# IIT-PAVIS/DiffAssemble

Hardware: AMD Instinct MI355X
Metric: denoising steps/sec (900-piece dense graph, T=100) (higher is better)
Workload: dtype bf16

## Files before the change

diffassemble_amd/_lib.py:

```python
import ctypes as C
import os

import torch

LIB_PATH = os.environ.get("DA_LIB_PATH") or os.path.join(os.path.dirname(os.path.abspath(__file__)), "lib", "libdiffassemble_hip.so")
DA_MAX_LAYERS = 8
ABI_VERSION = 19
PREC_F32, PREC_BF16 = 0, 1
VARIANT_2D, VARIANT_3D, VARIANT_DISCRETE = 0, 1, 2
ARCH_TRANSFORMER, ARCH_EXOPHORMER, ARCH_GCN = 0, 1, 2
MEAN_EPSILON, MEAN_START_X = 0, 1
ACT_NONE, ACT_GELU, ACT_LEAKY02 = 0, 1, 2
CONV_Q_PRESCALED, CONV_FOLDED_V32 = 1, 2
TRAIN_MMA_FP32, TRAIN_MMA_BF16 = 0, 1
TRAIN_BWD_ALL, TRAIN_BWD_EARLY, TRAIN_BWD_LATE = 0, 1, 2
D3PM_DRAW_SAMPLING, D3PM_DRAW_TRAINING = 0, 1
D3PM_LOSS = {"vb": 0, "cross_entropy": 1, "hybrid": 2}
DBG_COUNTERS = ("opt_gen_workgroups", "dense_fast_exits", "dual_gen_slabs", "opt_masked_gen_workgroups")
DBG_LAUNCH_COUNTERS = {"resident_launches": 4, "virtual_rows_in_launch": 5}
PROF_CLASSES = ("embed", "linear_mlp", "linear_qkvs", "attn_hidden", "attn_last", "head", "update", "conv_fused")

_fp = C.c_void_p
_FPL = _fp * DA_MAX_LAYERS


class DaWeights(C.Structure):
    _fields_ = [
        ("variant", C.c_int32), ("arch", C.c_int32), ("steps", C.c_int32), ("c_in", C.c_int32),
        ("c_out", C.c_int32), ("feat_dim", C.c_int32), ("hidden", C.c_int32), ("heads", C.c_int32),
        ("n_layers", C.c_int32), ("virt_nodes", C.c_int32),
        ("time_emb", _fp),
        ("pos_w0", _fp), ("pos_b0", _fp), ("pos_w1", _fp), ("pos_b1", _fp),
        ("mlp_w0", _fp), ("mlp_b0", _fp), ("mlp_w1", _fp), ("mlp_b1", _fp),
        ("conv_wq", _FPL), ("conv_bq", _FPL), ("conv_wk", _FPL), ("conv_bk", _FPL),
# ... 285 lines not shown
```

diffassemble_amd/csrc/da_api.hip:

```cpp
#include <stdarg.h>
#include <stdlib.h>
#include <string.h>

#include <utility>
#include <vector>

#include "da_common.h"
#include "da_internal.h"
#include "da_config.h"

namespace da {

static thread_local char g_err[1024] = "";

void set_error(const char *fmt, ...) {
    va_list ap;
    va_start(ap, fmt);
    vsnprintf(g_err, sizeof(g_err), fmt, ap);
    va_end(ap);
}

struct ConvW {
    void *w = nullptr;
    float *b = nullptr;
// ... 55 lines not shown
    float *mlp_b0 = nullptr, *mlp_b1 = nullptr;
    ConvW conv[DA_MAX_LAYERS];
    void *virt_emb = nullptr;
    void *head_w0 = nullptr;
    float *head_b0 = nullptr;
    float *head_w1 = nullptr, *head_b1 = nullptr, *head_r_w1 = nullptr, *head_r_b1 = nullptr;
    bool fused_mlp2 = false;
    void *conv0c_w = nullptr;
    float *conv0c_b = nullptr;
    void *headc_w = nullptr;
    float *headc_b = nullptr;
    void *virt_qkvs = nullptr;
    void *conv0c_wd = nullptr, *virt_qkvs_d = nullptr;
    void *conv0c_wdp = nullptr, *convLf_wp = nullptr;
    void *conv0c_wqs = nullptr;
    float *conv0c_bd = nullptr;
    bool q_prescaled = false;
    bool lastfold = false;
    bool dense_only = false;
    void *convLf_w = nullptr;
    float *convLf_b = nullptr;
    void *skipc_w = nullptr;
    float *skipc_b = nullptr;
    std::vector<void *> owned;
    bool prof_on = false;
    std::vector<hipEvent_t> prof_ev;
    std::vector<int> prof_cls;
    size_t prof_used = 0;
    struct LoopEntry { LoopKey a, b; hipGraphExec_t exec, exec_b; };
    std::vector<LoopEntry> loops;
// ... 332 lines not shown
                        DA_CHECK_HIP(hipStreamWaitEvent(st, d->ev_join, 0));
                        side_guard.armed = false;
                        xin = dst; ldx = c.hc;
                        continue;
                    }
                    rc = timed(d, last ? DA_PROF_ATTN_LAST : DA_PROF_ATTN_HIDDEN, st, [&] {
                        int r2 = launch_attn_dense(prec, L, d->heads, c.C, g->n_graphs, g->max_graph_nodes, g->graph_ptr,
                                                   g->pad_ptr, 0, resid, act, dst, st, &mk);
                        if (r2) return r2;
                        return launch_attn_csr_cont(prec, n, nr, g->agg_row_ptr ? g->agg_row_ptr : g->irr_row_ptr, g->agg_row_ptr ? g->agg_col_src : g->irr_col_src,
                                                    g->row_map, d->heads, c.C, g->n_pad, L, resid, act, dst, st, g->agg_row_ptr ? g->agg_mult : nullptr); });
                    if (rc) return rc < 0 ? 1 : rc;
                    xin = dst; ldx = c.hc;
                    continue;
                }
                rc = timed(d, last ? DA_PROF_ATTN_LAST : DA_PROF_ATTN_HIDDEN, st, [&] {
                    return launch_attn_dense(prec, L, d->heads, c.C, g->n_graphs, g->max_graph_nodes, g->graph_ptr,
                                             g->pad_ptr, g->dense == 2, resid, act, dst, st); });
                if (rc > 0) return rc;
                if (rc == 0) { xin = dst; ldx = c.hc; continue; }
            }
        }
        if ((rc = timed(d, DA_PROF_LINEAR_QKVS, st, [&] {
                 return linear(prec, nproj, c.din, 4 * c.hc, xin, ldx, c.w, c.b, DA_ACT_NONE, nullptr, w.qkvs, 4 * c.hc, st); }))) return rc;
        if (virt0 && (rc = launch_scatter_virtual(prec, n - nr, d->V, d->heads, c.C, d->virt_qkvs, nr, nullptr, 0, nullptr, nullptr,
                                                  nullptr, nullptr, w.qkvs, st))) return rc;
        DA_REQUIRE(g->row_ptr && (g->col_src || g->n_edges == 0), "da_graph: this call walks the edge list (alpha requested or no "
                   "MFMA attention for this layer) but the CSR arrays are missing");
        int tiny = -1;
        if (!al && g->dense && n == nr && g->graph_ptr && !dense_disabled()) {
            if ((rc = timed(d, last ? DA_PROF_ATTN_LAST : DA_PROF_ATTN_HIDDEN, st, [&] {
// ... 163 lines not shown
        void *p = nullptr;
        if (hipMalloc(&p, bytes < 256 ? 256 : bytes) != hipSuccess) { set_error("hipMalloc(%zu) failed", bytes); return nullptr; }
        d->owned.push_back(p);
        return p;
    };
    auto copy_f32 = [&](const float *src, size_t n) -> float * {
        float *p = (float *)alloc(n * 4);
        if (!p || hipMemcpyAsync(p, src, n * 4, hipMemcpyDeviceToDevice, st) != hipSuccess) { rc = 2; return nullptr; }
        return p;
    };
    auto pack = [&](const float *src, size_t n) -> void * {
        void *p = alloc(n * s + 4096);
        if (!p || launch_convert(precision, n, src, p, st)) { rc = 2; return nullptr; }
        return p;
    };
    auto pack_qs = [&](const void *wsrc, int K, int hc, int C) -> void * {
#ifndef DA_EXPERIMENTS
        return nullptr;
#endif
        if (precision != DA_PREC_BF16 || C != 32 || H != 8 || (K != 128 && K != 256) || !wsrc || mfma_disabled()) return nullptr;
        void *p = alloc(w_qs_bytes(H, K));
        if (!p || pack_w_qs(H, K, hc, wsrc, p, st)) { rc = 2; return nullptr; }
        return p;
    };
    auto pack_panel = [&](const void *wsrc, int K, int Nout) -> void * {
        const size_t nb = xpanel_in_model() ? da_linear_packed_bytes(precision, K, Nout) : 0;
        if (!nb || !wsrc) return nullptr;
        void *p = alloc(nb);
        if (!p || pack_w_xpanel(K, Nout, wsrc, K, p, st)) { rc = 2; return nullptr; }
        return p;
    };
    d->time_emb = copy_f32(w->time_emb, (size_t)w->steps * 32);
    if (discrete) {
        d->pos_w1 = copy_f32(w->pos_w1, (size_t)w->c_out * 32);
// ... 549 lines not shown
int da_conv_dense_ex(int prec, const da_graph *g, int heads, int C, int Din, const void *x, const void *w, const float *b,
                     const void *residual, int act, void *out, void *scratch, int flags, void *stream) {
    DA_REQUIRE(g && x && w && out && scratch, "da_conv_dense_ex: null argument");
    DA_REQUIRE(dense_ok(g, heads, C), "da_conv_dense_ex: graph is not dense or head width %d unsupported", C);
    const bool folded = (flags & DA_CONV_FOLDED_V32) != 0;
    DA_REQUIRE(!folded || (C == 144 && !residual && act == DA_ACT_NONE), "da_conv_dense_ex: folded value heads need C = 144, no residual, no activation");
    hipStream_t st = (hipStream_t)stream;
    const size_t s = esize(prec), hc = (size_t)heads * C;
    const size_t hb = align_up(((size_t)g->n_pad + 64) * hc * s, 256);
    char *base = (char *)scratch;
    QkvScatter qs;
    qs.HC = (int)hc; qs.C = C; qs.n_pad = g->n_pad; qs.row_map = g->row_map;
    qs.Q = base; qs.K = base + hb; qs.Vt = base + 2 * hb; qs.S = folded ? nullptr : base + 3 * hb;
    qs.Cv = folded ? 32 : 0;
    const int nout = folded ? 2 * (int)hc + heads * 32 : 4 * (int)hc;
    const bool qsf = !folded && !residual && !g->hybrid && g->n_nodes == g->n_real && b && w_qs_bytes(heads, Din) <= hb &&
                     attn_qsf_applicable(prec, heads, C, Din, g->n_graphs, g->max_graph_nodes, g->n_pad, (flags & DA_CONV_Q_PRESCALED) ? 1 : 0);
    void *wq_img = base + hb;
    int rc = 0;
    if (qsf) {
        if ((rc = pack_w_qs(heads, Din, (int)hc, w, wq_img, st))) return rc;
    } else
    rc = launch_gemm_mfma(prec, g->n_nodes, Din, nout, x, Din, w, b, DA_ACT_NONE, nullptr, nullptr, 0, &qs, st);
    DA_REQUIRE(rc == 0, "da_conv_dense_ex: projection shape (Din=%d, Nout=%d) not supported by the MFMA kernels", Din, nout);
    DenseLayout L;
    L.Q = qs.Q; L.K = qs.K; L.Vt = qs.Vt; L.S = qs.S; L.n_pad = g->n_pad; L.q_prescaled = (flags & DA_CONV_Q_PRESCALED) ? 1 : 0;
    if (qsf) { L.x = x; L.ldx = Din; L.kin = Din; L.wqs = wq_img; L.bias = b; }
    DenseFold fo;
    fo.cv = 32; fo.out = out; fo.n_rows = g->n_real;
    const DenseMask mk = dense_mask_of(g);
    rc = launch_attn_dense(prec, L, heads, C, g->n_graphs, g->max_graph_nodes, g->graph_ptr, g->pad_ptr, g->dense == 2, residual, act,
// ... 4 lines not shown

int da_debug_counters(int64_t *out, int n, int reset) {
    DA_REQUIRE(out && n >= DA_DBG_NCOUNTERS, "da_debug_counters: need room for %d counters", DA_DBG_NCOUNTERS);
    unsigned long long a[4] = {0, 0, 0, 0}, b2[2] = {0, 0};
    int rc;
    if ((rc = da::attn_dense_counters(a, reset))) return rc;
#ifdef DA_EXPERIMENTS
    if ((rc = da::attn_dual_counters(b2, reset))) return rc;
#endif
    for (int k = 0; k < n; ++k) out[k] = 0;
    out[DA_DBG_OPT_GEN_WORKGROUPS] = (int64_t)a[0];
    out[DA_DBG_DENSE_FAST_EXITS] = (int64_t)a[1];
    out[DA_DBG_DUAL_GEN_SLABS] = (int64_t)b2[0];
    out[DA_DBG_OPT_MASKED_GEN_WORKGROUPS] = (int64_t)a[2];
    out[DA_DBG_RES_LAUNCHES] = (int64_t)da::attn_res_launches(reset);
    out[DA_DBG_VIRT_IN_LAUNCH] = (int64_t)da::attn_virt_launches(reset);
    return 0;
}

int da_profile_enable(da_denoiser *d, int on) {
    DA_REQUIRE(d, "da_profile_enable: null denoiser");
    d->prof_on = on != 0;
    d->prof_used = 0;
    d->prof_cls.clear();
    return 0;
}

int da_profile_read(da_denoiser *d, float *ms, int32_t *counts) {
    DA_REQUIRE(d && ms && counts, "da_profile_read: null argument");
    for (int k = 0; k < DA_PROF_NCLASS; ++k) { ms[k] = 0.f; counts[k] = 0; }
// ... 54 lines not shown
```

diffassemble_amd/csrc/da_attn_dense.hip:

```cpp
#include <stdlib.h>

#include "da_attn_common.h"

namespace da {

#ifdef DA_ATTN_PROBE
#define DA_ATTN_DBG(...) __VA_ARGS__
#define DA_TICK(var) const unsigned long long var = __builtin_readcyclecounter()
#else
#define DA_ATTN_DBG(...)
#define DA_TICK(var)
#endif

__device__ unsigned long long g_attn_fallbacks[4];

template <typename T, int C, bool MASKED, int CV, int NST, int NW>
__global__ __launch_bounds__(64 * NW, (sizeof(T) == 4 && C == 144 && CV == 144) ? 1 : 2) void k_attn_dense(AttnDenseParams p) {
    using CF = Cfg<T, C, CV>;
    constexpr int QT = 32 * NW, NT = 64 * NW, MAXI = (CF::NI + NW - 1) / NW;
    extern __shared__ __attribute__((aligned(16))) unsigned char smem[];

    float *mlut = (float *)(smem + NST * CF::STAGE);
    if (MASKED && threadIdx.x < 64) {
        const int e = threadIdx.x >> 2, b = threadIdx.x & 3;
// ... 743 lines not shown
#ifdef DA_EXPERIMENTS
    if (prec == DA_PREC_BF16 && C == 32 && !p.mask && attn2_env() DA_ATTN_DBG(&& !p.debug && !p.prof))
        return launch_attn_dense2(p, heads, n_graphs, max_graph_nodes, st);
#endif
    if (prec == DA_PREC_BF16) return C == 32 ? launch_tc<bf16_t, 32>(p, st) : launch_tc<bf16_t, 144>(p, st);
    return C == 32 ? launch_tc<float, 32>(p, st) : launch_tc<float, 144>(p, st);
}

bool attn_res_qsf_shape_ok(int max_nodes, int n_pad, int n_graphs, int kin);
bool attn_qsf_applicable(int prec, int heads, int C, int kin, int n_graphs, int max_graph_nodes, int n_pad, int q_prescaled) {
    if (prec != DA_PREC_BF16 || heads != 8 || C != 32 || !q_prescaled || !attn_opt_env()) return false;
    if (DA_XENV("DA_ATTN_NO_FAST", 0) DA_ATTN_DBG(|| DA_XENV_LIVE("DA_ATTN_DEBUG") || DA_XENV_LIVE("DA_ATTN_PROF_PTR"))) return false;
    if ((size_t)C * (size_t)n_pad * 2 >= ((size_t)1 << 31)) return false;
    return attn_res_qsf_shape_ok(max_graph_nodes, n_pad, n_graphs, kin);
}

int attn_dense_counters(unsigned long long *out4, int reset) {
    DA_CHECK_HIP(hipMemcpyFromSymbol(out4, HIP_SYMBOL(g_attn_fallbacks), 4 * sizeof(unsigned long long)));
    if (reset) { const unsigned long long z[4] = {0, 0, 0, 0}; DA_CHECK_HIP(hipMemcpyToSymbol(HIP_SYMBOL(g_attn_fallbacks), z, sizeof(z))); }
    unsigned long long o2[2] = {0, 0};
    const int rc = attn_opt_counters(o2, reset);
    if (rc) return rc;
    out4[0] = o2[0];
    out4[2] = o2[1];
    return 0;
}

}
```

diffassemble_amd/csrc/da_attn_opt.hip:

```cpp
#include <stdlib.h>

#include <type_traits>

#include "da_attn_common.h"
#include "da_attn_res_asm.inc"

namespace da {

#ifdef DA_OPT_PROBE
#define DA_OPB(...) __VA_ARGS__
#else
#define DA_OPB(...)
#endif

__device__ unsigned long long g_opt_fallbacks[2];

__device__ __forceinline__ void virt_rows_block(const AttnDenseParams &p, int vb, unsigned char *smem) {
    constexpr int EPL = 4, U = 4, C = 32;
    const int row = vb / p.v_split, part = vb - row * p.v_split;
    const int i = p.v_n_real + row;
    const int beg = p.v_row_ptr[i], end = p.v_row_ptr[i + 1];
    const int lane = threadIdx.x & 63, wv = threadIdx.x >> 6;
    const int head = lane >> 3, sub = (lane & 7) * EPL;
    const size_t hb = (size_t)head * (size_t)p.n_pad;
// ... 722 lines not shown
    int grid = p.nqt * p.H * p.n_graphs;
    t_virt_taken = false;
    if constexpr (C == 32 && !FOLD && MASKED && NWV == 4) {
        if (p.v_rows > 0) {
            p.v_split = p.v_n_real >= 8192 ? DA_VIRT_SPLIT_MAX : 4;
            grid += (p.v_rows * p.v_split + 7) & ~7;
            t_virt_taken = true;
            __atomic_fetch_add(&g_virt_launches, 1ll, __ATOMIC_RELAXED);
        }
    } else {
        p.v_rows = 0;
    }
    k_attn_optt<C, FOLD, MASKED, NST, MINB, BK, VAR, NWV><<<grid, 64 * NWV, lds, st>>>(p);
    DA_LAUNCH_CHECK();
    return 0;
}

template <int NWV, bool QUEUE, bool KPF, int XV = 0>
__global__ __launch_bounds__(64 * NWV, NWV >= 16 ? 1 : ((NWV > 5 || (XV & 8)) ? 4 : 5)) void k_attn_res(AttnDenseParams p) {
    constexpr bool O2 = (XV & 1) != 0, PROG = (XV & 16) != 0, MSK = (XV & 32) != 0, QSF = (XV & 64) != 0, PIPE2 = (XV & 256) != 0;
    static_assert(!PIPE2 || (NWV == 16 && KPF && !PROG && !MSK && !O2), "pipelined key loop: the sixteen-wave instances on complete graphs");
    static_assert(!QSF || (NWV == 16 && KPF && QUEUE && !PROG && !MSK && !O2), "projection in the prologue: the sixteen-wave default instance");
    static_assert(!MSK || (NWV == 16 && KPF && !PROG && !O2), "masked resident instance: sixteen waves, K fragments one block ahead");
    static_assert(!PROG || (NWV == 16 && KPF), "progressive landing: the sixteen-wave instance (two waves per piece index), K fragments one block ahead");
    using T = bf16_t;
    constexpr int C = 32, CV = 32;
    using CF = Cfg<T, C, CV, 64>;
    using KG = OptK<C, 64>;
    static_assert(KG::NI == 8, "eight 1 KB pieces per 64-key stage");
    static_assert(CF::ROWB == 64 && CF::ROWBV == 64 && KG::RS == 64 && CF::RSV == 64 && KG::KBYTES == 4096, "one tile stride for K and V; 2 KB per 32-key block");
// ... 12 lines not shown
    const size_t np = (size_t)p.n_pad;
    const unsigned char *Qg = (const unsigned char *)p.Q + ((size_t)h * np + pad0) * CF::ROWB;
    const unsigned char *Kg = (const unsigned char *)p.K + ((size_t)h * np + pad0) * CF::ROWB;
    const unsigned char *Vg = (const unsigned char *)p.Vt + ((size_t)h * np + pad0) * CF::ROWBV;
    const unsigned lds0 = (unsigned)(size_t)(__attribute__((address_space(3))) unsigned char *)smem;
    unsigned *qctr = (unsigned *)(smem + ((p.max_nodes + 63) >> 6) * STAGE);
    volatile unsigned *land = qctr + 4;
    float *mlut = (float *)(qctr + 36);
    if (MSK && tid < 64) mlut[tid] = (((tid >> 2) >> (tid & 3)) & 1) ? 0.f : -INFINITY;
    constexpr int KS = QSF ? ((XV & 128) ? 8 : 16) : 1;
    [[maybe_unused]] unsigned char *wimg = (unsigned char *)qctr + 512;
    [[maybe_unused]] float *biasl = (float *)(wimg + 2 * KS * 1024);
    if constexpr (QSF) {
        const unsigned char *wsrc = (const unsigned char *)p.wqs + (size_t)h * 4 * KS * 1024;
        const unsigned wl = lds0 + (unsigned)(wimg - smem);
        const int qs_off = ((p.max_nodes + 63) >> 6) * STAGE - 2 * KS * 1024;
        for (int j = wid; j < 4 * KS; j += NWV) {
            const int blk = j / KS, s_ = j - blk * KS;
            const unsigned dst = (blk == 1 || blk == 2) ? wl + (unsigned)(((blk - 1) * KS + s_) * 1024) : lds0 + (unsigned)(qs_off + ((blk ? 1 : 0) * KS + s_) * 1024);
            asm volatile("s_mov_b32 m0, %0\n\ts_nop 0\n\tglobal_load_lds_dwordx4 %1, %2" ::"s"(dst), "v"((unsigned)lane * 16u), "s"(wsrc + (size_t)j * 1024) : "memory");
        }
        if (tid < 128) biasl[tid] = (tid < 32 ? p.bias_q : (tid < 64 ? p.bias_k : (tid < 96 ? p.bias_v : p.bias_s)))[32 * h + (tid & 31)];
    }
    if (QUEUE && tid == 0) { *qctr = 0u; asm volatile("s_waitcnt lgkmcnt(0)" ::: "memory"); }
    if (PROG && tid < 32) { land[tid] = 0u; asm volatile("s_waitcnt lgkmcnt(0)" ::: "memory"); }
    int node0 = 0, n_g = 0;
    if (!upad) { node0 = p.graph_ptr[g]; n_g = p.graph_ptr[g + 1] - node0; }
    const int nkt = upad ? (npg >> 6) : ((n_g + 63) >> 6);
    u32x4 qf0[2] = {};
    if constexpr (PROG) {
        const unsigned char *qrow = Qg + (size_t)(wid * 32 + i) * CF::ROWB + half * 16;
// ... 43 lines not shown
            const int32_t *gpp = p.graph_ptr + g;
            asm volatile("s_load_dwordx2 %0, %1, 0x0\n\ts_waitcnt lgkmcnt(0)" : "=s"(gp2) : "s"(gpp) : "memory");
            node0 = gp2[0]; n_g = gp2[1] - gp2[0];
        } else { node0 = p.graph_ptr[g]; n_g = p.graph_ptr[g + 1] - node0; }
    }
    const int nslab = (n_g + 31) >> 5;
    int slab = wid;
    u32x4 qf[CF::NCH];
    auto load_q = [&](int sl, u32x4(&dst)[CF::NCH]) {
        const unsigned char *qrow = Qg + (size_t)(max(min(sl, nslab - 1), 0) * 32 + i) * CF::ROWB;
#pragma unroll
        for (int ch = 0; ch < CF::NCH; ++ch) dst[ch] = *(const u32x4 *)(qrow + ch * 32 + half * 16);
    };
    static_assert(!PROG || CF::NCH == 2, "progressive landing: two Q fragments per lane");
    [[maybe_unused]] u32x4 xq[KS];
    [[maybe_unused]] auto x_issue = [&](int sl) {
        const int nd = max(min(sl * 32 + i, n_g - 1), 0);
        const unsigned char *row = (const unsigned char *)p.x + ((size_t)(node0 + nd) * (size_t)p.ldx + 8 * half) * 2;
        if (p.debug == 77) row = (const unsigned char *)p.x + ((size_t)(node0 + max(min(sl * 32, n_g - 32), 0)) * (size_t)p.ldx) * 2 + lane * 16;
#pragma unroll
        for (int s_ = 0; s_ < KS; ++s_) xq[s_] = *(const u32x4 *)(row + s_ * (p.debug == 77 ? 1024 : 32));
    };
    [[maybe_unused]] auto chain2 = [&](const unsigned char *w0b, const unsigned char *w1b, f32x16 &a0, f32x16 &a1) {
        unsigned lo = (unsigned)lane * 16u;
        asm volatile("" : "+v"(lo));
#pragma unroll
        for (int r = 0; r < 16; ++r) { a0[r] = 0.f; a1[r] = 0.f; }
        u32x4 wa0 = *(const u32x4 *)(w0b + lo), wa1 = *(const u32x4 *)(w1b + lo);
#pragma unroll
        for (int s_ = 0; s_ < KS; ++s_) {
            u32x4 wn0 = wa0, wn1 = wa1;
            if (s_ + 1 < KS) { wn0 = *(const u32x4 *)(w0b + (size_t)(s_ + 1) * 1024 + lo); wn1 = *(const u32x4 *)(w1b + (size_t)(s_ + 1) * 1024 + lo); }
            __builtin_amdgcn_sched_barrier(0);
            a0 = __builtin_amdgcn_mfma_f32_32x32x16_bf16(__builtin_bit_cast(bf16x8, wa0), __builtin_bit_cast(bf16x8, xq[s_]), a0, 0, 0, 0);
            a1 = __builtin_amdgcn_mfma_f32_32x32x16_bf16(__builtin_bit_cast(bf16x8, wa1), __builtin_bit_cast(bf16x8, xq[s_]), a1, 0, 0, 0);
            __builtin_amdgcn_sched_barrier(0);
            wa0 = wn0; wa1 = wn1;
        }
    };
    [[maybe_unused]] auto chunk_of = [&](const f32x16 &a, int blk, int t) {
        const f32x4 b0 = *(const f32x4 *)(biasl + 32 * blk + 16 * t + 8 * half), b1 = *(const f32x4 *)(biasl + 32 * blk + 16 * t + 8 * half + 4);
        bf16x8 q8;
#pragma unroll
        for (int e = 0; e < 4; ++e) { q8[e] = (__bf16)(a[8 * t + e] + b0[e]); q8[4 + e] = (__bf16)(a[8 * t + 4 + e] + b1[e]); }
        return __builtin_bit_cast(u32x4, q8);
    };
    [[maybe_unused]] auto project_qs = [&](int sl, bool keep) {
        f32x16 aQ, aS;
        const unsigned char *wq_ = smem + (size_t)(((p.max_nodes + 63) >> 6) * STAGE - 2 * KS * 1024);
        chain2(wq_, wq_ + (size_t)KS * 1024, aQ, aS);
        const int row = sl * 32 + i;
#pragma unroll
        for (int t = 0; t < 2; ++t) {
            const u32x4 qc = chunk_of(aQ, 0, t), sc_ = chunk_of(aS, 3, t);
            if (keep) qf[t] = qc;
            if (row < n_g) {
                *(u32x4 *)(const_cast<unsigned char *>(Qg) + (size_t)row * CF::ROWB + (2 * t + half) * 16) = qc;
                *(u32x4 *)((unsigned char *)p.S + ((size_t)(node0 + row) * HC + (size_t)h * C) * 2 + (2 * t + half) * 16) = sc_;
            }
        }
    };
    [[maybe_unused]] auto project_kv = [&](int sl) {
        f32x16 aK, aV;
        chain2(wimg, wimg + (size_t)KS * 1024, aK, aV);
        const int rt = (sl & 1) * 32 + i;
        unsigned char *st_ = smem + (size_t)(sl >> 1) * STAGE + (size_t)rt * 64;
#pragma unroll
        for (int t = 0; t < 2; ++t) {
            *(u32x4 *)(st_ + (((2 * t + half) ^ KG::f(rt)) << 4)) = chunk_of(aK, 1, t);
            *(u32x4 *)(st_ + KG::KBYTES + ((2 * t + half) << 4)) = chunk_of(aV, 2, t);
        }
    };
    if constexpr (QSF) x_issue(slab);
    else if constexpr (!PROG) load_q(slab, qf);    else if constexpr (!PROG) load_q(slab, qf);
    [[maybe_unused]] const int t0p = wid >> 3, nmine = nkt > t0p ? (nkt - t0p + 1) >> 1 : 0;
    [[maybe_unused]] int posted = 0;
    [[maybe_unused]] auto wait_le = [&](int n) {
        switch (n) {
            case 0: asm volatile("s_waitcnt vmcnt(0)" ::: "memory"); break;
            case 1: asm volatile("s_waitcnt vmcnt(1)" ::: "memory"); break;
            case 2: asm volatile("s_waitcnt vmcnt(2)" ::: "memory"); break;
            case 3: asm volatile("s_waitcnt vmcnt(3)" ::: "memory"); break;
            case 4: asm volatile("s_waitcnt vmcnt(4)" ::: "memory"); break;
            case 5: asm volatile("s_waitcnt vmcnt(5)" ::: "memory"); break;
            case 6: asm volatile("s_waitcnt vmcnt(6)" ::: "memory"); break;
            case 7: asm volatile("s_waitcnt vmcnt(7)" ::: "memory"); break;
            case 8: asm volatile("s_waitcnt vmcnt(8)" ::: "memory"); break;
            default: asm volatile("s_waitcnt vmcnt(9)" ::: "memory"); break;
        }
// ... 15 lines not shown
        } while (true);
    };
    if constexpr (PROG) {
        __builtin_amdgcn_s_barrier();
        post_upto(slab < nslab ? 1 : (1 << 30));
        if (nmine == 0) asm volatile("s_waitcnt vmcnt(0)" ::: "memory");
        qf[0] = qf0[0]; qf[1] = qf0[1];
        asm volatile("" : "+v"(qf[0]), "+v"(qf[1]));
        if (slab < nslab) await_tile(0);
    } else {
    if constexpr (QSF) {
        const int slabB = slab + NWV;
        const bool hasA = slab < nslab, hasB = slabB < nslab;
        asm volatile("s_waitcnt vmcnt(0) lgkmcnt(0)" ::: "memory");
        __builtin_amdgcn_s_barrier();
        if (hasA) { project_qs(slab, true); project_kv(slab); }
        if (hasB) { x_issue(slabB); project_qs(slabB, false); }
        __builtin_amdgcn_s_barrier();
        if (hasB) project_kv(slabB);
        asm volatile("s_waitcnt vmcnt(0) lgkmcnt(0)" ::: "memory");
        __builtin_amdgcn_s_barrier();
    } else {
    asm volatile("s_waitcnt vmcnt(0)" : "+v"(qf[0]), "+v"(qf[CF::NCH - 1]));
    __builtin_amdgcn_s_barrier();
    }
    }
    DA_OPB(pb_[6] = __builtin_readcyclecounter();)

    const int pi_i = (i & 3) + 4 * ((i >> 3) & 3) + 16 * ((i >> 2) & 1);
    int kfo[CF::NCH];
#pragma unroll
    for (int ch = 0; ch < CF::NCH; ++ch) kfo[ch] = pi_i * KG::RS + (((2 * ch + half) ^ KG::f(pi_i)) * 16);
    const int li = lane & 15;
    const unsigned vbase = lds0 + (unsigned)(KG::KBYTES + (16 * half + (li >> 2)) * CF::RSV + (16 * ((lane >> 4) & 1) + 4 * (li & 3)) * 2);
// ... 345 lines not shown
#pragma unroll
            for (int ch = 0; ch < CF::NCH; ++ch) qf[ch] = qn[ch];
            asm volatile("" : "+v"(qf[0]), "+v"(qf[CF::NCH - 1]));
        }
        slab = nxt;
        DA_OPB({ if (round < 2) pb_[3 + 2 * round] = __builtin_readcyclecounter(); })
    }
    DA_OPB({ if (p.prof && lane == 0) { pb_[7] = __builtin_readcyclecounter(); unsigned long long *o_ = p.prof + ((size_t)blockIdx.x * NWV + wid) * 8;
             for (int k = 0; k < 8; ++k) o_[k] = pb_[k]; } })
}

static long long g_res_launches = 0;
long long attn_res_launches(int reset) {
    return reset ? __atomic_exchange_n(&g_res_launches, 0ll, __ATOMIC_RELAXED) : __atomic_load_n(&g_res_launches, __ATOMIC_RELAXED);
}

static size_t attn_res_qsf_lds(int max_nodes, int kin) { return (size_t)((max_nodes + 63) >> 6) * OptK<32, 64>::STAGE + 512 + (size_t)2 * (kin >> 4) * 1024 + 512; }
static bool attn_res_takes(int max_nodes, int n_pad, int n_graphs) {
    return cfg().attn_level >= 2 && DA_XENV("DA_OPT_HID", 0) == 0 && max_nodes >= DA_XENV("DA_ATTN_RES_MIN", 512) && max_nodes <= 19 * 64 &&
           (long long)n_pad * 2 >= (long long)n_graphs * max_nodes;
}
bool attn_res_qsf_shape_ok(int max_nodes, int n_pad, int n_graphs, int kin) {
#ifndef DA_EXPERIMENTS
    return false;
#endif
    if (!DA_XENV("DA_ATTN_RES_QSF", 0) || (kin != 128 && kin != 256)) return false;
    if (DA_XENV("DA_ATTN_RES_PH", 1) != 1) return false;
    return attn_res_takes(max_nodes, n_pad, n_graphs) && attn_res_qsf_lds(max_nodes, kin) <= (size_t)160 * 1024 &&
           (size_t)((max_nodes + 63) >> 6) * OptK<32, 64>::STAGE >= (size_t)8 * OptK<32, 64>::STAGE + (size_t)2 * (kin >> 4) * 1024;
}

__global__ void k_pack_w_qs(int heads, int kin, int hc, const bf16_t *__restrict__ W, u32x4 *__restrict__ out) {
    const int KS = kin >> 4;
    const size_t idx = (size_t)blockIdx.x * blockDim.x + threadIdx.x, total = (size_t)heads * 4 * KS * 64;
    if (idx >= total) return;
    const int lane = (int)(idx & 63), s = (int)((idx >> 6) % KS), hm = (int)((idx >> 6) / KS), m = hm & 3, h = hm >> 2;
    const int a = lane & 31, row = (a & 0x13) | (((a >> 2) & 1) << 3) | (((a >> 3) & 1) << 2);
    out[idx] = *(const u32x4 *)(W + ((size_t)m * hc + 32 * h + row) * kin + 16 * s + 8 * (lane >> 5));
}
size_t w_qs_bytes(int heads, int kin) { return (size_t)heads * 4 * kin * 64; }
int pack_w_qs(int heads, int kin, int hc, const void *wd, void *packed, hipStream_t st) {
    const size_t total = w_qs_bytes(heads, kin) / 16;
    k_pack_w_qs<<<(unsigned)((total + 255) / 256), 256, 0, st>>>(heads, kin, hc, (const bf16_t *)wd, (u32x4 *)packed);
    DA_LAUNCH_CHECK();
// ... 34 lines not shown
                (long long)p.n_pad * 2 >= (long long)p.n_graphs * p.max_nodes)
                return launch_res<16, true, true, 32>(p, st);
#endif
            return launch_optt<32, false, true, 4, 4>(p, st);
        }
        [[maybe_unused]] const int v = DA_XENV("DA_OPT_HID", 0);
        {
            const int res = cfg().attn_level >= 2, res_min = DA_XENV("DA_ATTN_RES_MIN", 512);
#ifdef DA_EXPERIMENTS
            const int res_small = DA_XENV("DA_ATTN_RES_SMALL", 0);
            if (res && res_small && v == 0 && p.max_nodes > 128 && p.max_nodes <= 160 && (long long)p.n_pad * 2 >= (long long)p.n_graphs * p.max_nodes)
                return res_small == 2 ? launch_res<5, false, true, 8>(p, st)
                                      : launch_res<5, false, true>(p, st);
#endif
            if (res && v == 0 && p.max_nodes >= res_min && p.max_nodes <= 19 * 64  && (long long)p.n_pad * 2 >= (long long)p.n_graphs * p.max_nodes) {
#ifdef DA_EXPERIMENTS
                if (p.x) {
                    DA_REQUIRE(attn_res_qsf_shape_ok(p.max_nodes, p.n_pad, p.n_graphs, p.kin) && p.wqs && p.bias_q && p.bias_k && p.bias_v && p.bias_s,
                               "k_attn_res: projection in the prologue requested for a shape it does not take");
                    return p.kin == 256 ? launch_res<16, true, true, 64>(p, st) : launch_res<16, true, true, 64 + 128>(p, st);
                }
#endif
#ifdef DA_EXPERIMENTS
                switch (DA_XENV("DA_ATTN_RES_PH", 1)) {
                    case 3: return launch_res<16, false, true>(p, st);
                    case 4: return launch_res<16, true, false>(p, st);
                    case 5: return launch_res<16, true, true, 1>(p, st);
                    case 6: return launch_res<16, true, true, 2>(p, st);
                    case 7: return launch_res<16, true, true, 3>(p, st);
                    case 8: return launch_res<16, true, true, 16>(p, st);
                    default: break;
                }
#endif
#ifdef DA_EXPERIMENTS
                switch (DA_XENV("DA_ATTN_RES_PIPE", 0)) {
                    case 1: return launch_res<16, true, true, 256>(p, st);
                    case 2: return launch_res<16, true, true, 256 + 512 * 1>(p, st);
// ... 87 lines not shown
```

diffassemble_amd/csrc/da_config.h:

```cpp
#pragma once
#include <stdlib.h>

#include "../../include/diffassemble_hip.h"

namespace da {

da_config &cfg();

enum { DA_FOLD_MLP2 = 1, DA_FOLD_LAST = 2, DA_FOLD_QSCALE = 4, DA_FOLD_DDIM = 8, DA_FOLD_TAIL = 16, DA_FOLD_HYBRID_OVERLAP = 32 };

#ifdef DA_EXPERIMENTS
inline int xenv_read(const char *name, int dflt) { const char *e = getenv(name); return e ? atoi(e) : dflt; }
#define DA_XENV(name, dflt) ([]() -> int { static const int v_ = da::xenv_read(name, dflt); return v_; }())
#define DA_XENV_LIVE(name) getenv(name)
#define DA_XENV_SET(name) (getenv(name) != nullptr)
#else
#define DA_XENV(name, dflt) (dflt)
#define DA_XENV_LIVE(name) ((const char *)nullptr)
#define DA_XENV_SET(name) (false)
#endif

}
```

diffassemble_amd/csrc/da_internal.h:

```cpp
#pragma once
#include "da_common.h"
#include "da_config.h"

namespace da {

struct DeviceSchedule {
    int steps;
    const float *betas, *alphas_cumprod, *sqrt_recip_alphas, *sqrt_recip_alphas_cumprod,
        *sqrt_recipm1_alphas_cumprod, *sqrt_one_minus_alphas_cumprod, *posterior_variance;
};

__device__ __forceinline__ float ddim2d_value(const DeviceSchedule &s, int mean_type, long long ti, int ratio,
                                              int prev_all_nonneg, float eta, float xv, float m, float noise) {
    ti = ti < 0 ? 0 : (ti >= s.steps ? s.steps - 1 : ti);
    const long long tp = ti - ratio;
    const float ap = s.alphas_cumprod[ti];
    const float ap_prev = (prev_all_nonneg && tp >= 0) ? s.alphas_cumprod[tp] : 1.0f;
    const float beta = 1.0f - ap;
    const float x0 = mean_type == DA_MEAN_START_X ? m : (xv - sqrtf(beta) * m) / sqrtf(ap);
    const float eps = (s.sqrt_recip_alphas_cumprod[ti] * xv - x0) / s.sqrt_recipm1_alphas_cumprod[ti];
    const float var = ((1.0f - ap_prev) / (1.0f - ap)) * (1.0f - ap / ap_prev);
    const float std_eta = eta * sqrtf(var);
    float prev = sqrtf(ap_prev) * x0 + sqrtf(1.0f - ap_prev - std_eta * std_eta) * eps;
    if (eta > 0.f) prev += std_eta * noise;
// ... 91 lines not shown
    int Cv = 0;
    int blocks = 0;
    const int32_t *row_map;
    void *Q, *K, *Vt, *S;
};
struct DenseLayout {
    const void *Q, *K, *Vt, *S;
    int n_pad;
    int q_prescaled = 0;
    const void *x = nullptr;
    int ldx = 0, kin = 0;
    const void *wqs = nullptr;
    const float *bias = nullptr;
};
bool attn_qsf_applicable(int prec, int heads, int C, int kin, int n_graphs, int max_graph_nodes, int n_pad, int q_prescaled);
size_t w_qs_bytes(int heads, int kin);
int pack_w_qs(int heads, int kin, int hc, const void *wd, void *packed, hipStream_t st);
int launch_gemm_mfma(int prec, int M, int K, int Nout, const void *A, int lda, const void *W, const float *bias,
                     int act, const void *res, void *out, int ldo, const QkvScatter *qs, hipStream_t st, int ldw = 0,
                     const void *pre = nullptr, const void *wpacked = nullptr);
size_t xpanel_packed_bytes(int K, int Nout);
bool xpanel_in_model();
void gemm_thin_set(int v);
int xpanel_mode();
int pack_w_xpanel(int K, int Nout, const void *W, int ldw, void *packed, hipStream_t st);
struct DenseMask {
    const uint8_t *mask;
    const int64_t *mask_ptr;
    const int32_t *irr_row_ptr, *irr_col_src, *row_map;
    const int32_t *slot_node = nullptr;
// ... 19 lines not shown
    return mk;
}
struct DenseFold {
    int cv;
    void *out;
    int n_rows;
};
int launch_attn_dense(int prec, const DenseLayout &L, int heads, int C, int n_graphs, int max_graph_nodes,
                      const int32_t *graph_ptr, const int32_t *pad_ptr, int nodiag, const void *res, int act,
                      void *out, hipStream_t st, const DenseMask *mk = nullptr, const DenseFold *fold = nullptr);
int launch_attn_dual(const DenseLayout &L, int heads, int C, int n_graphs, int max_graph_nodes, const int32_t *graph_ptr,
                     const int32_t *pad_ptr, int nodiag, int act, void *out, const DenseFold *fold, hipStream_t st);
int attn_dense_counters(unsigned long long *out4, int reset);
long long attn_virt_launches(int reset);
long long attn_res_launches(int reset);
int attn_dual_counters(unsigned long long *out2, int reset);
int launch_attn_csr_cont(int prec, int n_nodes, int n_real, const int32_t *irr_row_ptr, const int32_t *irr_col_src,
                         const int32_t *row_map, int heads, int C, int n_pad, const DenseLayout &L,
                         const void *residual, int act, void *out, hipStream_t st,
                         const float *mult = nullptr );

bool conv_fused_applicable(int prec, int heads, int C, int kin, int max_graph_nodes, int ldo);
int launch_conv_fused(int prec, int heads, int C, int kin, int n_graphs, int max_graph_nodes, const int32_t *graph_ptr,
                      int nodiag, const void *x, int ldx, const void *W, const float *bias, int act, void *out, int ldo,
                      hipStream_t st);

int pcd_knn_launch(int clouds, int N, int dim, const float *x, int ldx, int32_t *idx, const float *xn, hipStream_t st);
int pcd_premap_launch(int C, const float *X, int ldx, const float *Wm, long long total, float *T, hipStream_t st);
int pcd_edge_launch(const float *T, const int32_t *idx, const float *bn_a, const float *wb, int N, int clouds, float *Xout,
                    float *xn, hipStream_t st);
// ... 50 lines not shown
```

include/diffassemble_hip.h:

```cpp
#ifndef DIFFASSEMBLE_HIP_H
#define DIFFASSEMBLE_HIP_H

#include <stddef.h>
#include <stdint.h>

#ifdef __cplusplus
extern "C" {
#endif

#define DA_ABI_VERSION 19

enum { DA_PREC_F32 = 0, DA_PREC_BF16 = 1 };
enum { DA_VARIANT_2D = 0, DA_VARIANT_3D = 1,
       DA_VARIANT_DISCRETE = 2 };
enum { DA_ARCH_TRANSFORMER = 0, DA_ARCH_EXOPHORMER = 1,
       DA_ARCH_GCN = 2 };
enum { DA_MEAN_EPSILON = 0, DA_MEAN_START_X = 1 };
enum { DA_ACT_NONE = 0, DA_ACT_GELU = 1, DA_ACT_LEAKY02 = 2 };
enum { DA_MAX_LAYERS = 8 };

int da_abi_version(void);
const char *da_last_error(void);

typedef struct da_config {
// ... 203 lines not shown
                  const float *b, const void *residual, int act, void *out, void *scratch, void *stream);

#define DA_CONV_Q_PRESCALED 1
#define DA_CONV_FOLDED_V32 2
int da_conv_dense_ex(int prec, const da_graph *g, int heads, int C, int Din, const void *x, const void *w,
                     const float *b, const void *residual, int act, void *out, void *scratch, int flags,
                     void *stream);

enum {
    DA_DBG_OPT_GEN_WORKGROUPS = 0,
    DA_DBG_DENSE_FAST_EXITS = 1,
    DA_DBG_DUAL_GEN_SLABS = 2,
    DA_DBG_OPT_MASKED_GEN_WORKGROUPS = 3,
    DA_DBG_RES_LAUNCHES = 4,
    DA_DBG_VIRT_IN_LAUNCH = 5,
    DA_DBG_NCOUNTERS = 8
};
int da_debug_counters(int64_t *out , int n, int reset);

size_t da_train_workspace_bytes(const da_weights *w, const da_graph *g);
size_t da_train_workspace_bytes_ex(const da_weights *w, const da_graph *g, int mma_precision);
#define DA_TRAIN_MMA_FP32 0
#define DA_TRAIN_MMA_BF16 1
int da_train_forward(const da_weights *w, const da_graph *g, const float *x, const int64_t *t,
                     const float *feats, float *out, void *workspace, size_t workspace_bytes,
                     void *stream);
int da_train_backward(const da_weights *w, const da_weights *grads, const da_graph *g, const float *x,
                      const int64_t *t, const float *d_out, float *d_feats, void *workspace,
                      size_t workspace_bytes, void *stream);
int da_train_forward_ex(const da_weights *w, const da_graph *g, const float *x, const int64_t *t,
// ... 209 lines not shown
```

Measured before the change: 94340.

## Enable fused QKVS projection in resident attention kernel prologue by default

Turns on, by default, the path that computes the Q/K/V/S projections inside the resident dense attention kernel instead of running a separate linear launch. It also restructures the in-kernel projection into single-accumulator MFMA chains that reload the next slab's X rows during the V chain, and moves the packed weight image in LDS so smaller graphs fit. The aim is to remove the separate QKVS GEMM launch and its global-memory round trip. The trade-offs are added LDS pressure and register scheduling changes, plus an opt-out flag and a launch counter.

```diff
diff --git a/diffassemble_amd/_lib.py b/diffassemble_amd/_lib.py
--- a/diffassemble_amd/_lib.py
+++ b/diffassemble_amd/_lib.py
@@ -17,7 +17,8 @@
 D3PM_DRAW_SAMPLING, D3PM_DRAW_TRAINING = 0, 1
 D3PM_LOSS = {"vb": 0, "cross_entropy": 1, "hybrid": 2}
 DBG_COUNTERS = ("opt_gen_workgroups", "dense_fast_exits", "dual_gen_slabs", "opt_masked_gen_workgroups")
-DBG_LAUNCH_COUNTERS = {"resident_launches": 4, "virtual_rows_in_launch": 5}
+DBG_LAUNCH_COUNTERS = {"resident_launches": 4, "virtual_rows_in_launch": 5,
+                       "resident_projection_launches": 6}
 PROF_CLASSES = ("embed", "linear_mlp", "linear_qkvs", "attn_hidden", "attn_last", "head", "update", "conv_fused")
 
 _fp = C.c_void_p
diff --git a/diffassemble_amd/csrc/da_api.hip b/diffassemble_amd/csrc/da_api.hip
--- a/diffassemble_amd/csrc/da_api.hip
+++ b/diffassemble_amd/csrc/da_api.hip
@@ -93,6 +93,7 @@
     void *conv0c_wd = nullptr, *virt_qkvs_d = nullptr;
     void *conv0c_wdp = nullptr, *convLf_wp = nullptr;
     void *conv0c_wqs = nullptr;
+    bool attn_qsf = false;
     float *conv0c_bd = nullptr;
     bool q_prescaled = false;
     bool lastfold = false;
@@ -455,7 +456,7 @@
                     xin = dst; ldx = c.hc;
                     continue;
                 }
-                rc = timed(d, last ? DA_PROF_ATTN_LAST : DA_PROF_ATTN_HIDDEN, st, [&] {
+                rc = timed(d, qsf ? DA_PROF_CONV_FUSED : (last ? DA_PROF_ATTN_LAST : DA_PROF_ATTN_HIDDEN), st, [&] {
                     return launch_attn_dense(prec, L, d->heads, c.C, g->n_graphs, g->max_graph_nodes, g->graph_ptr,
                                              g->pad_ptr, g->dense == 2, resid, act, dst, st); });
                 if (rc > 0) return rc;
@@ -649,10 +650,9 @@
         if (!p || launch_convert(precision, n, src, p, st)) { rc = 2; return nullptr; }
         return p;
     };
+    d->attn_qsf = attn_qsf_enabled();
     auto pack_qs = [&](const void *wsrc, int K, int hc, int C) -> void * {
-#ifndef DA_EXPERIMENTS
-        return nullptr;
-#endif
+        if (!d->attn_qsf) return nullptr;
         if (precision != DA_PREC_BF16 || C != 32 || H != 8 || (K != 128 && K != 256) || !wsrc || mfma_disabled()) return nullptr;
         void *p = alloc(w_qs_bytes(H, K));
         if (!p || pack_w_qs(H, K, hc, wsrc, p, st)) { rc = 2; return nullptr; }
@@ -1232,7 +1232,7 @@
     qs.Q = base; qs.K = base + hb; qs.Vt = base + 2 * hb; qs.S = folded ? nullptr : base + 3 * hb;
     qs.Cv = folded ? 32 : 0;
     const int nout = folded ? 2 * (int)hc + heads * 32 : 4 * (int)hc;
-    const bool qsf = !folded && !residual && !g->hybrid && g->n_nodes == g->n_real && b && w_qs_bytes(heads, Din) <= hb &&
+    const bool qsf = attn_qsf_enabled() && !folded && !residual && !g->hybrid && g->n_nodes == g->n_real && b && w_qs_bytes(heads, Din) <= 2 * hb &&
                      attn_qsf_applicable(prec, heads, C, Din, g->n_graphs, g->max_graph_nodes, g->n_pad, (flags & DA_CONV_Q_PRESCALED) ? 1 : 0);
     void *wq_img = base + hb;
     int rc = 0;
@@ -1267,6 +1267,7 @@
     out[DA_DBG_DUAL_GEN_SLABS] = (int64_t)b2[0];
     out[DA_DBG_OPT_MASKED_GEN_WORKGROUPS] = (int64_t)a[2];
     out[DA_DBG_RES_LAUNCHES] = (int64_t)da::attn_res_launches(reset);
+    out[DA_DBG_RES_PROJ_LAUNCHES] = (int64_t)da::attn_res_qsf_launches(reset);
     out[DA_DBG_VIRT_IN_LAUNCH] = (int64_t)da::attn_virt_launches(reset);
     return 0;
 }
diff --git a/diffassemble_amd/csrc/da_attn_dense.hip b/diffassemble_amd/csrc/da_attn_dense.hip
--- a/diffassemble_amd/csrc/da_attn_dense.hip
+++ b/diffassemble_amd/csrc/da_attn_dense.hip
@@ -781,6 +781,10 @@
     if ((size_t)C * (size_t)n_pad * 2 >= ((size_t)1 << 31)) return false;
     return attn_res_qsf_shape_ok(max_graph_nodes, n_pad, n_graphs, kin);
 }
+bool attn_qsf_enabled() {
+    const int x = DA_XENV("DA_ATTN_RES_QSF", -1);
+    return x < 0 ? !(cfg().disable_folds & DA_FOLD_ATTN_PROJ) : x != 0;
+}
 
 int attn_dense_counters(unsigned long long *out4, int reset) {
     DA_CHECK_HIP(hipMemcpyFromSymbol(out4, HIP_SYMBOL(g_attn_fallbacks), 4 * sizeof(unsigned long long)));
diff --git a/diffassemble_amd/csrc/da_attn_opt.hip b/diffassemble_amd/csrc/da_attn_opt.hip
--- a/diffassemble_amd/csrc/da_attn_opt.hip
+++ b/diffassemble_amd/csrc/da_attn_opt.hip
@@ -760,6 +760,12 @@
     k_attn_optt<C, FOLD, MASKED, NST, MINB, BK, VAR, NWV><<<grid, 64 * NWV, lds, st>>>(p);
     DA_LAUNCH_CHECK();
     return 0;
+}
+
+template <int KS>
+__host__ __device__ static inline int res_qsf_qs_off(int max_nodes) {
+    const int img = ((max_nodes + 63) >> 6) * OptK<32, 64>::STAGE;
+    return img >= 8 * OptK<32, 64>::STAGE + 2 * KS * 1024 ? img - 2 * KS * 1024 : img + 512 + 2 * KS * 1024 + 512;
 }
 
 template <int NWV, bool QUEUE, bool KPF, int XV = 0>
@@ -802,7 +808,7 @@
     if constexpr (QSF) {
         const unsigned char *wsrc = (const unsigned char *)p.wqs + (size_t)h * 4 * KS * 1024;
         const unsigned wl = lds0 + (unsigned)(wimg - smem);
-        const int qs_off = ((p.max_nodes + 63) >> 6) * STAGE - 2 * KS * 1024;
+        const int qs_off = res_qsf_qs_off<KS>(p.max_nodes);
         for (int j = wid; j < 4 * KS; j += NWV) {
             const int blk = j / KS, s_ = j - blk * KS;
             const unsigned dst = (blk == 1 || blk == 2) ? wl + (unsigned)(((blk - 1) * KS + s_) * 1024) : lds0 + (unsigned)(qs_off + ((blk ? 1 : 0) * KS + s_) * 1024);
@@ -876,28 +882,40 @@
     };
     static_assert(!PROG || CF::NCH == 2, "progressive landing: two Q fragments per lane");
     [[maybe_unused]] u32x4 xq[KS];
-    [[maybe_unused]] auto x_issue = [&](int sl) {
+    [[maybe_unused]] const int xstep = p.debug == 77 ? 1024 : 32;
+    [[maybe_unused]] auto x_row = [&](int sl) {
         const int nd = max(min(sl * 32 + i, n_g - 1), 0);
         const unsigned char *row = (const unsigned char *)p.x + ((size_t)(node0 + nd) * (size_t)p.ldx + 8 * half) * 2;
         if (p.debug == 77) row = (const unsigned char *)p.x + ((size_t)(node0 + max(min(sl * 32, n_g - 32), 0)) * (size_t)p.ldx) * 2 + lane * 16;
-#pragma unroll
-        for (int s_ = 0; s_ < KS; ++s_) xq[s_] = *(const u32x4 *)(row + s_ * (p.debug == 77 ? 1024 : 32));
+        return row;
     };
-    [[maybe_unused]] auto chain2 = [&](const unsigned char *w0b, const unsigned char *w1b, f32x16 &a0, f32x16 &a1) {
+    [[maybe_unused]] auto x_issue = [&](int sl) {
+        const unsigned char *row = x_row(sl);
+#pragma unroll
+        for (int s_ = 0; s_ < KS; ++s_) xq[s_] = *(const u32x4 *)(row + s_ * xstep);
+    };
+    struct Reload { enum { value = 1 }; };
+    struct NoReload { enum { value = 0 }; };
+    typedef const __attribute__((address_space(1))) u32x4 *xptr_t;
+    [[maybe_unused]] auto chain1 = [&](auto rl, const unsigned char *wb, f32x16 &a, const unsigned char *nxt = nullptr) {
         unsigned lo = (unsigned)lane * 16u;
         asm volatile("" : "+v"(lo));
 #pragma unroll
-        for (int r = 0; r < 16; ++r) { a0[r] = 0.f; a1[r] = 0.f; }
-        u32x4 wa0 = *(const u32x4 *)(w0b + lo), wa1 = *(const u32x4 *)(w1b + lo);
+        for (int r = 0; r < 16; ++r) a[r] = 0.f;
+        u32x4 wa = *(const u32x4 *)(wb + lo);
 #pragma unroll
         for (int s_ = 0; s_ < KS; ++s_) {
-            u32x4 wn0 = wa0, wn1 = wa1;
-            if (s_ + 1 < KS) { wn0 = *(const u32x4 *)(w0b + (size_t)(s_ + 1) * 1024 + lo); wn1 = *(const u32x4 *)(w1b + (size_t)(s_ + 1) * 1024 + lo); }
+            u32x4 wn = wa;
+            if (s_ + 1 < KS) wn = *(const u32x4 *)(wb + (size_t)(s_ + 1) * 1024 + lo);
             __builtin_amdgcn_sched_barrier(0);
-            a0 = __builtin_amdgcn_mfma_f32_32x32x16_bf16(__builtin_bit_cast(bf16x8, wa0), __builtin_bit_cast(bf16x8, xq[s_]), a0, 0, 0, 0);
-            a1 = __builtin_amdgcn_mfma_f32_32x32x16_bf16(__builtin_bit_cast(bf16x8, wa1), __builtin_bit_cast(bf16x8, xq[s_]), a1, 0, 0, 0);
+            a = __builtin_amdgcn_mfma_f32_32x32x16_bf16(__builtin_bit_cast(bf16x8, wa), __builtin_bit_cast(bf16x8, xq[s_]), a, 0, 0, 0);
             __builtin_amdgcn_sched_barrier(0);
-            wa0 = wn0; wa1 = wn1;
+            if constexpr (decltype(rl)::value) {
+                asm volatile("" : "+v"(nxt));
+                xq[s_] = *(xptr_t)(size_t)nxt;
+                nxt += xstep;
+            }
+            wa = wn;
         }
     };
     [[maybe_unused]] auto chunk_of = [&](const f32x16 &a, int blk, int t) {
@@ -908,33 +926,36 @@
         return __builtin_bit_cast(u32x4, q8);
     };
     [[maybe_unused]] auto project_qs = [&](int sl, bool keep) {
-        f32x16 aQ, aS;
-        const unsigned char *wq_ = smem + (size_t)(((p.max_nodes + 63) >> 6) * STAGE - 2 * KS * 1024);
-        chain2(wq_, wq_ + (size_t)KS * 1024, aQ, aS);
+        const unsigned char *wq_ = smem + (size_t)res_qsf_qs_off<KS>(p.max_nodes);
         const int row = sl * 32 + i;
+        f32x16 a;
+        chain1(NoReload(), wq_, a);
 #pragma unroll
         for (int t = 0; t < 2; ++t) {
-            const u32x4 qc = chunk_of(aQ, 0, t), sc_ = chunk_of(aS, 3, t);
+            const u32x4 qc = chunk_of(a, 0, t);
             if (keep) qf[t] = qc;
-            if (row < n_g) {
-                *(u32x4 *)(const_cast<unsigned char *>(Qg) + (size_t)row * CF::ROWB + (2 * t + half) * 16) = qc;
-                *(u32x4 *)((unsigned char *)p.S + ((size_t)(node0 + row) * HC + (size_t)h * C) * 2 + (2 * t + half) * 16) = sc_;
-            }
+            if (row < n_g) *(u32x4 *)(const_cast<unsigned char *>(Qg) + (size_t)row * CF::ROWB + (2 * t + half) * 16) = qc;
+        }
+        chain1(NoReload(), wq_ + (size_t)KS * 1024, a);
+#pragma unroll
+        for (int t = 0; t < 2; ++t) {
+            const u32x4 sc_ = chunk_of(a, 3, t);
+            if (row < n_g) *(u32x4 *)((unsigned char *)p.S + ((size_t)(node0 + row) * HC + (size_t)h * C) * 2 + (2 * t + half) * 16) = sc_;
         }
     };
-    [[maybe_unused]] auto project_kv = [&](int sl) {
-        f32x16 aK, aV;
-        chain2(wimg, wimg + (size_t)KS * 1024, aK, aV);
+    [[maybe_unused]] auto project_kv = [&](auto rl, int sl, const unsigned char *nxt = nullptr) {
         const int rt = (sl & 1) * 32 + i;
         unsigned char *st_ = smem + (size_t)(sl >> 1) * STAGE + (size_t)rt * 64;
-#pragma unroll
-        for (int t = 0; t < 2; ++t) {
-            *(u32x4 *)(st_ + (((2 * t + half) ^ KG::f(rt)) << 4)) = chunk_of(aK, 1, t);
-            *(u32x4 *)(st_ + KG::KBYTES + ((2 * t + half) << 4)) = chunk_of(aV, 2, t);
-        }
+        f32x16 a;
+        chain1(NoReload(), wimg, a);
+#pragma unroll
+        for (int t = 0; t < 2; ++t) *(u32x4 *)(st_ + (((2 * t + half) ^ KG::f(rt)) << 4)) = chunk_of(a, 1, t);
+        chain1(rl, wimg + (size_t)KS * 1024, a, nxt);
+#pragma unroll
+        for (int t = 0; t < 2; ++t) *(u32x4 *)(st_ + KG::KBYTES + ((2 * t + half) << 4)) = chunk_of(a, 2, t);
     };
-    if constexpr (QSF) x_issue(slab);
-    else if constexpr (!PROG) load_q(slab, qf);    else if constexpr (!PROG) load_q(slab, qf);
+    if constexpr (QSF) { if (slab < nslab) x_issue(slab); }
+    else if constexpr (!PROG) load_q(slab, qf);
     [[maybe_unused]] const int t0p = wid >> 3, nmine = nkt > t0p ? (nkt - t0p + 1) >> 1 : 0;
     [[maybe_unused]] int posted = 0;
     [[maybe_unused]] auto wait_le = [&](int n) {
@@ -980,10 +1001,13 @@
         const bool hasA = slab < nslab, hasB = slabB < nslab;
         asm volatile("s_waitcnt vmcnt(0) lgkmcnt(0)" ::: "memory");
         __builtin_amdgcn_s_barrier();
-        if (hasA) { project_qs(slab, true); project_kv(slab); }
-        if (hasB) { x_issue(slabB); project_qs(slabB, false); }
+        if (hasA) {
+            project_qs(slab, true);
+            if (hasB) { project_kv(Reload(), slab, x_row(slabB)); project_qs(slabB, false); }
+            else project_kv(NoReload(), slab);
+        }
         __builtin_amdgcn_s_barrier();
-        if (hasB) project_kv(slabB);
+        if (hasB) project_kv(NoReload(), slabB);
         asm volatile("s_waitcnt vmcnt(0) lgkmcnt(0)" ::: "memory");
         __builtin_amdgcn_s_barrier();
     } else {
@@ -1359,20 +1383,24 @@
 long long attn_res_launches(int reset) {
     return reset ? __atomic_exchange_n(&g_res_launches, 0ll, __ATOMIC_RELAXED) : __atomic_load_n(&g_res_launches, __ATOMIC_RELAXED);
 }
-
-static size_t attn_res_qsf_lds(int max_nodes, int kin) { return (size_t)((max_nodes + 63) >> 6) * OptK<32, 64>::STAGE + 512 + (size_t)2 * (kin >> 4) * 1024 + 512; }
+static long long g_res_qsf_launches = 0;
+long long attn_res_qsf_launches(int reset) {
+    return reset ? __atomic_exchange_n(&g_res_qsf_launches, 0ll, __ATOMIC_RELAXED) : __atomic_load_n(&g_res_qsf_launches, __ATOMIC_RELAXED);
+}
+
+static size_t attn_res_qsf_lds(int max_nodes, int kin) {
+    const size_t img = (size_t)((max_nodes + 63) >> 6) * OptK<32, 64>::STAGE, wb = (size_t)2 * (kin >> 4) * 1024, base = img + 512 + wb + 512;
+    const size_t qs = (size_t)(kin == 128 ? res_qsf_qs_off<8>(max_nodes) : res_qsf_qs_off<16>(max_nodes));
+    return qs >= img ? qs + wb : base;
+}
 static bool attn_res_takes(int max_nodes, int n_pad, int n_graphs) {
     return cfg().attn_level >= 2 && DA_XENV("DA_OPT_HID", 0) == 0 && max_nodes >= DA_XENV("DA_ATTN_RES_MIN", 512) && max_nodes <= 19 * 64 &&
            (long long)n_pad * 2 >= (long long)n_graphs * max_nodes;
 }
 bool attn_res_qsf_shape_ok(int max_nodes, int n_pad, int n_graphs, int kin) {
-#ifndef DA_EXPERIMENTS
-    return false;
-#endif
-    if (!DA_XENV("DA_ATTN_RES_QSF", 0) || (kin != 128 && kin != 256)) return false;
-    if (DA_XENV("DA_ATTN_RES_PH", 1) != 1) return false;
-    return attn_res_takes(max_nodes, n_pad, n_graphs) && attn_res_qsf_lds(max_nodes, kin) <= (size_t)160 * 1024 &&
-           (size_t)((max_nodes + 63) >> 6) * OptK<32, 64>::STAGE >= (size_t)8 * OptK<32, 64>::STAGE + (size_t)2 * (kin >> 4) * 1024;
+    if (kin != 128 && kin != 256) return false;
+    if (DA_XENV("DA_ATTN_RES_PH", 1) != 1 || DA_XENV("DA_ATTN_RES_PIPE", 0) != 0) return false;
+    return attn_res_takes(max_nodes, n_pad, n_graphs) && attn_res_qsf_lds(max_nodes, kin) <= (size_t)160 * 1024;
 }
 
 __global__ void k_pack_w_qs(int heads, int kin, int hc, const bf16_t *__restrict__ W, u32x4 *__restrict__ out) {
@@ -1437,13 +1465,12 @@
                                       : launch_res<5, false, true>(p, st);
 #endif
             if (res && v == 0 && p.max_nodes >= res_min && p.max_nodes <= 19 * 64  && (long long)p.n_pad * 2 >= (long long)p.n_graphs * p.max_nodes) {
-#ifdef DA_EXPERIMENTS
                 if (p.x) {
                     DA_REQUIRE(attn_res_qsf_shape_ok(p.max_nodes, p.n_pad, p.n_graphs, p.kin) && p.wqs && p.bias_q && p.bias_k && p.bias_v && p.bias_s,
                                "k_attn_res: projection in the prologue requested for a shape it does not take");
+                    __atomic_fetch_add(&g_res_qsf_launches, 1ll, __ATOMIC_RELAXED);
                     return p.kin == 256 ? launch_res<16, true, true, 64>(p, st) : launch_res<16, true, true, 64 + 128>(p, st);
                 }
-#endif
 #ifdef DA_EXPERIMENTS
                 switch (DA_XENV("DA_ATTN_RES_PH", 1)) {
                     case 3: return launch_res<16, false, true>(p, st);
diff --git a/diffassemble_amd/csrc/da_config.h b/diffassemble_amd/csrc/da_config.h
--- a/diffassemble_amd/csrc/da_config.h
+++ b/diffassemble_amd/csrc/da_config.h
@@ -7,7 +7,7 @@
 
 da_config &cfg();
 
-enum { DA_FOLD_MLP2 = 1, DA_FOLD_LAST = 2, DA_FOLD_QSCALE = 4, DA_FOLD_DDIM = 8, DA_FOLD_TAIL = 16, DA_FOLD_HYBRID_OVERLAP = 32 };
+enum { DA_FOLD_MLP2 = 1, DA_FOLD_LAST = 2, DA_FOLD_QSCALE = 4, DA_FOLD_DDIM = 8, DA_FOLD_TAIL = 16, DA_FOLD_HYBRID_OVERLAP = 32, DA_FOLD_ATTN_PROJ = 64 };
 
 #ifdef DA_EXPERIMENTS
 inline int xenv_read(const char *name, int dflt) { const char *e = getenv(name); return e ? atoi(e) : dflt; }
diff --git a/diffassemble_amd/csrc/da_internal.h b/diffassemble_amd/csrc/da_internal.h
--- a/diffassemble_amd/csrc/da_internal.h
+++ b/diffassemble_amd/csrc/da_internal.h
@@ -129,6 +129,7 @@
     const float *bias = nullptr;
 };
 bool attn_qsf_applicable(int prec, int heads, int C, int kin, int n_graphs, int max_graph_nodes, int n_pad, int q_prescaled);
+bool attn_qsf_enabled();
 size_t w_qs_bytes(int heads, int kin);
 int pack_w_qs(int heads, int kin, int hc, const void *wd, void *packed, hipStream_t st);
 int launch_gemm_mfma(int prec, int M, int K, int Nout, const void *A, int lda, const void *W, const float *bias,
@@ -178,6 +179,7 @@
 int attn_dense_counters(unsigned long long *out4, int reset);
 long long attn_virt_launches(int reset);
 long long attn_res_launches(int reset);
+long long attn_res_qsf_launches(int reset);
 int attn_dual_counters(unsigned long long *out2, int reset);
 int launch_attn_csr_cont(int prec, int n_nodes, int n_real, const int32_t *irr_row_ptr, const int32_t *irr_col_src,
                          const int32_t *row_map, int heads, int C, int n_pad, const DenseLayout &L,
diff --git a/include/diffassemble_hip.h b/include/diffassemble_hip.h
--- a/include/diffassemble_hip.h
+++ b/include/diffassemble_hip.h
@@ -241,6 +241,7 @@
     DA_DBG_OPT_MASKED_GEN_WORKGROUPS = 3,
     DA_DBG_RES_LAUNCHES = 4,
     DA_DBG_VIRT_IN_LAUNCH = 5,
+    DA_DBG_RES_PROJ_LAUNCHES = 6,
     DA_DBG_NCOUNTERS = 8
 };
 int da_debug_counters(int64_t *out , int n, int reset);
```

New measurement: 98140, median of 6. +4.0%, better.
